# dsteinberg/libcluster

Hardware: AMD Instinct MI355X
Metric: E-step data-points/sec (full VBEM iteration: suff-stats + M-step + E-step) (higher is better)
Workload: dtype f64

## Files before the change

### libcluster_amd/csrc/lc_kernels.h

```cpp
#pragma once
#include <hip/hip_runtime.h>
#include <cstdint>

namespace lck {

constexpr int RG = 16;

inline int padded_dim(int D) {
  return D <= 16 ? 16 : D <= 32 ? 32 : D <= 48 ? 48 : D <= 64 ? 64 : D <= 80 ? 80 : D <= 96 ? 96 : D <= 112 ? 112 : D <= 128 ? 128 : -1;
}
__host__ __device__ constexpr int lds_row_stride(int DP) { return DP == 16 ? 16 : (DP + 16) % 32 != 16 ? DP + 32 : DP + 16; }
inline int padded_dim_wide(int D) { return D <= 128 ? padded_dim(D) : (D + 63) / 64 * 64; }
constexpr int GW_MAX_DP = 1024;
inline int ntiles(int DP) { int nt = DP / 4; return nt * (nt + 1) / 2; }
inline int pstride(int DP) { return ntiles(DP) * 16 + DP; }
constexpr int WIDE_CHUNK = 256 * 16 + 64;
inline int wide_chunks(int DP) { int np = DP / 64; return np * (np + 1) / 2; }
inline int64_t estep_pstride(int DP, int DC) { return DP > 128 ? (int64_t)wide_chunks(DP) * WIDE_CHUNK : (int64_t)pstride(DC); }
inline int64_t estep_pstride(int DP) { return estep_pstride(DP, DP); }
inline int estep_active_width(int D, int DP) {
  if (DP < 32 || DP > 128) return DP;
  const int g = DP <= 48 ? 4 : 8, lo = DP <= 48 ? DP - 12 : DP - 8;
  const int dc = (D + g - 1) / g * g;
  return dc < DP ? (dc < lo ? lo : dc) : DP;
}
inline int64_t stat_stride(int DP) { return 1 + (int64_t)DP + (int64_t)DP * DP; }

struct LdsGrant {
  size_t granted[16] = {};
};
inline hipError_t grant_dynamic_lds(const void* fn, size_t bytes, LdsGrant& g) {
  if (bytes <= 64 * 1024) return hipSuccess;
  int dev = -1;
  const bool tracked = hipGetDevice(&dev) == hipSuccess && dev >= 0 && dev < 16;
  if (tracked && bytes <= g.granted[dev]) return hipSuccess;
  const hipError_t e = hipFuncSetAttribute(fn, hipFuncAttributeMaxDynamicSharedMemorySize, (int)bytes);
  if (e == hipSuccess && tracked) g.granted[dev] = bytes;
  return e;
}

inline int rginfo_pack(int group, int nvalid) { return (group << 5) | nvalid; }

struct EstepLaunch {
  int DP;
  int DC = 0;
  const double* X;
  int64_t nrg;
  const int* rginfo;
  int64_t nrows;
  const double* params;
  const double* ctab;
  int K;
  double* qZ;
  int64_t ldq;
  double* fz_part;
  double* ll_part;
  int raw = 0;
  int sparse = 0;
  int lq_lds = 0;
};
struct EstepPlan {
  bool ok;
  int rows_per_block;
  int64_t grid;
  bool four_groups;
  int DC, lq_lds;
  size_t lds_bytes;
};
EstepPlan estep_plan(const EstepLaunch& a);
int64_t estep_grid(const EstepLaunch& a);
hipError_t launch_estep(const EstepLaunch& a, hipStream_t stream);

struct FusedLaunch {
  int DP;
  int D = 16;
  const double* X;
  int64_t nrg;
  const int* rginfo;
  int64_t nrows;
  const double* params;
  const double* ctab;
  int K;
  double* qZ;
  int64_t ldq;
  double* partial;
  bool want_ll;
  int grid;
  int ngroups = 1;
  int yshare = 0;
};
constexpr int FUSED_CT_CAP = 1024;
inline int64_t fused_record(int DP, int K) { return (int64_t)K * (1 + DP + (int64_t)DP * DP) + 1 + K; }
bool fused_eligible(int DP, int K);
int fused_plan(int DP, int64_t nrg, int K);
hipError_t launch_fused(const FusedLaunch& a, hipStream_t stream);

struct SSItem {
  int64_t r0, r1;
  int kofs, kcnt;
  int64_t rec0;
};
constexpr int SS_BR = 32;
constexpr double SPECK_TAU = 0x1p-300;
enum SuffstatRoute { SS_PER_CLUSTER = 0, SS_FEAT = 1, SS_QUAD = 2, SS_WIDE = 3 };
enum SuffstatMode { SS_DENSE = 0, SS_MASKED_DENSE = 1, SS_ZERO_SKIP = 2, SS_WORK_LIST = 3 };
struct SuffstatPlan {
  SuffstatRoute route;
  int nchunks;
  int64_t chunk_rows;
  int extra, klast0, KR;
  int clusters_per_block;
  const char* name;
};
SuffstatPlan suffstat_plan(int DP, int DC, int64_t NP, int K, SuffstatMode mode);
struct SuffstatLaunch {
  int DP;
  int DC = 0;
  const double* X;
  int64_t NP;
  const double* qZ;
  int64_t ldq;
  int K;
  SuffstatMode mode = SS_DENSE;
  const int* rginfo;
  const unsigned char* smask;
  double* partial;
  int nchunks = 0, KR = 0;
  int64_t chunk_rows = 0;
  const SSItem* items = nullptr;
  const int* klist = nullptr;
  int nitems = 0, skip_listed = 0;
  int speck_skip = 0;
  int nslice = 1;
  int slice0 = 0, rs = 1, klast0 = 0, nklast = 0;
  int64_t ldx = 0;
  int DPW = 0, colA = 0, colB = 0;
};
hipError_t launch_suffstat(const SuffstatLaunch& a, const SuffstatPlan& p, hipStream_t stream);

constexpr int SPECK_PROBE_STEPS = 4096;
constexpr int64_t SPECK_PROBE_MIN_ROWS = 4096;
hipError_t launch_speck_probe(const double* qZ, int64_t ldq, int K, int64_t NP, int* active, int64_t* pairs, hipStream_t stream,
                              int64_t* rows = nullptr);
inline bool speck_probe_says_skip(int64_t active, int64_t pairs) { return pairs > 0 && 4 * (pairs - active) >= pairs; }
bool speck_probe_says_lists(int64_t single, int64_t rows);

struct SsListLayout {
  int nq;
  bool wide;
  size_t ent_off;
  size_t bytes;
};
inline SsListLayout ss_list_layout(int nchunks, int64_t chunk_rows, int K) {
  SsListLayout l{(K + 3) / 4, chunk_rows > 65536, 0, 0};
  l.ent_off = ((size_t)nchunks * l.nq * sizeof(int) + 15) / 16 * 16;
  l.bytes = l.ent_off + (size_t)nchunks * l.nq * (size_t)chunk_rows * (l.wide ? 4 : 2);
  return l;
}
bool suffstat_list_instance(int DP, int DC);
bool speck_lists_enabled();
hipError_t launch_suffstat_list_build(const SuffstatLaunch& a, const SuffstatPlan& p, void* lists, size_t bytes, hipStream_t stream);
hipError_t launch_suffstat_lists(const SuffstatLaunch& a, const SuffstatPlan& p, void* lists, size_t bytes, hipStream_t stream);
int speck_skip_mode();

__host__ __device__ constexpr int ft_offdiag(int DC) { return (DC / 4) * (DC / 4 - 1) / 2; }
__host__ __device__ constexpr int ft_features(int DC) { return 16 * ft_offdiag(DC) + 10 * (DC / 4) + DC + 1; }
__host__ __device__ constexpr int ft_tiles(int DC) { return (ft_features(DC) + 15) / 16; }
enum FtKind { FT_PRODUCT = 0, FT_LINEAR = 1, FT_COUNT = 2, FT_SPARE = 3 };
struct FtFeature {
  int u, w, kind;
};
__host__ __device__ __attribute__((always_inline)) constexpr FtFeature ft_feature(int DC, int one, int f) {
  const int noff = 16 * ft_offdiag(DC), ndiag = 10 * (DC / 4);
  if (f < noff) {
    const int p = f / 16, r = f % 16;
    int ja = 1;
    while ((ja + 1) * ja / 2 <= p) ++ja;
    return {4 * (p - ja * (ja - 1) / 2) + (r & 3), 4 * ja + (r >> 2), FT_PRODUCT};
  }
  f -= noff;
  if (f < ndiag) {
    const int b = 4 * (f / 10), e = f % 10;
    const int i = e < 4 ? 0 : e < 7 ? 1 : e < 9 ? 2 : 3, i0 = e < 4 ? 0 : e < 7 ? 4 : e < 9 ? 7 : 9;
    return {b + i, b + i + (e - i0), FT_PRODUCT};
  }
  f -= ndiag;
  if (f < DC) return {f, one, FT_LINEAR};
  return {one, one, f == DC ? FT_COUNT : FT_SPARE};
}
#ifndef LC_FT_WAVES64
#define LC_FT_WAVES64 8
#endif
#ifndef LC_FT_WAVES128
#define LC_FT_WAVES128 8
#endif
__host__ __device__ constexpr int ft_waves(int DP) { return DP == 64 ? LC_FT_WAVES64 : DP == 128 ? LC_FT_WAVES128 : DP > 64 ? 8 : 4; }
__host__ __device__ constexpr int ft_tpw_max(int DP, int NQ) {
  const int t = (NQ >= 8 && DP > 64 && DP < 128 ? 64 : 72) / NQ;
  return t < 14 ? t : 14;
}
__host__ __device__ constexpr int ft_nslice(int DP, int DC, int NQ) {
  return (ft_tiles(DC) + ft_waves(DP) * ft_tpw_max(DP, NQ) - 1) / (ft_waves(DP) * ft_tpw_max(DP, NQ));
}
__host__ __device__ constexpr int ft_tpw(int DP, int DC, int NQ) {
  return (ft_tiles(DC) + ft_waves(DP) * ft_nslice(DP, DC, NQ) - 1) / (ft_waves(DP) * ft_nslice(DP, DC, NQ));
}
__host__ __device__ __attribute__((always_inline)) constexpr void ft_deal(int DP, int DC, int NQ, int slice, int wave, int* t0, int* nt) {
  const int tiles = ft_tiles(DC), nsl = ft_nslice(DP, DC, NQ);
  if (ft_waves(DP) == 8) {
    const int ns = 4 * nsl, s = slice * 4 + (wave & 3), l = tiles / ns, r = tiles % ns;
    const int load = l + (s < r ? 1 : 0), first = s * l + (s < r ? s : r);
    *t0 = first + (wave < 4 ? 0 : (load + 1) / 2);
    *nt = wave < 4 ? (load + 1) / 2 : load / 2;
  } else {
    const int tpw = ft_tpw(DP, DC, NQ), t = (slice * 4 + wave) * tpw;
    *t0 = t;
    *nt = tiles - t < tpw ? (tiles - t > 0 ? tiles - t : 0) : tpw;
  }
}
__host__ __device__ constexpr int ftl_tpw(int DC) { return ((ft_tiles(DC) + 3) / 4 + 1) / 2; }
__host__ __device__ __attribute__((always_inline)) constexpr void ft_deal_one(int DC, int wave, int* t0, int* nt) {
  const int tiles = ft_tiles(DC), s = wave & 3, l = tiles / 4, r = tiles % 4;
  const int load = l + (s < r ? 1 : 0), first = s * l + (s < r ? s : r);
  *t0 = first + (wave < 4 ? 0 : (load + 1) / 2);
  *nt = wave < 4 ? (load + 1) / 2 : load / 2;
}
__host__ __device__ constexpr int ft_nt_min(int DP, int DC, int NQ) {
  int m = ft_tpw(DP, DC, NQ);
  for (int sl = 0; sl < ft_nslice(DP, DC, NQ); ++sl)
    for (int w = 0; w < ft_waves(DP); ++w) {
      int t0 = 0, nt = 0;
      ft_deal(DP, DC, NQ, sl, w, &t0, &nt);
      m = nt < m ? nt : m;
    }
  return m;
}

hipError_t launch_fold_extra(double* rec, int64_t SS, int K, int klast0, int extra, hipStream_t stream);
hipError_t launch_reduce_records(const double* partial, int64_t n, int K, const int* kptr, const int* krec, double* out,
                                 hipStream_t stream);

constexpr int REDUCE_TMP_ELEMS = 512;
hipError_t launch_reduce_partials(const double* partial, int nparts, int64_t n, double* out, hipStream_t stream,
                                  double* tmp = nullptr);
hipError_t launch_group_colsum(const double* qZ, int64_t ldq, int K, const int64_t* goff, int J, double* out,
                               hipStream_t stream, double* tmp = nullptr, int64_t rows = 0);
hipError_t launch_fill_qz(double* qZ, int64_t ldq, int K, const int* rginfo, int64_t nrows, int64_t nrg, double value,
                          hipStream_t stream);
struct DiagEstepLaunch {
  int DP, D;
  const double* X;
  int64_t nrg;
  const int* rginfo;
  int64_t nrows;
  const double* params;
  int mode = 0;
  const double* ctab;
  int K;
  double* qZ;
  int64_t ldq;
  double* fz_part;
  double* ll_part;
  int raw = 0;
  const double* wt = nullptr;
  const double* mu = nullptr;
  const double* constk = nullptr;
  int ngroups = 1;
  double* sink = nullptr;
};
constexpr int EDM_CT_CAP = 1024;
inline int64_t estep_diag_grid(int64_t nrg) { return (nrg * RG + 63) / 64; }
int64_t estep_diag_mfma_weights(int DP, int K, int mode);
enum DiagEstepInstance { EDI_NONE = 0, EDI_GENERIC = 1, EDI_PLAIN = 2, EDI_TABLED = 3, EDI_ONEGROUP = 4 };
struct DiagEstepPlan {
  bool ok;
  bool mfma;
  int mode;
  int64_t grid;
  size_t lds_bytes;
  const char* name;
  bool wide;
  int KT;
  bool REG;
  int NT;
  bool QUAD;
  int R, KTM;
  int instance;
  int64_t nslots;
  int per_cu;
  int64_t block_cap;
};
DiagEstepPlan estep_diag_plan(const DiagEstepLaunch& a);
hipError_t launch_estep_diag(const DiagEstepLaunch& a, hipStream_t stream);
double estep_diag_centre(int D, int DP, int K, int mode, const double* a, const double* w2, double* mu);
void estep_diag_pack(int D, int DP, int K, int mode, const double* a, const double* w2, const double* w1, const double* mu,
                     double* constk, double* wt, int64_t nw);

struct DiagStatLaunch {
  int DP;
  const double* X;
  int64_t NP;
  const double* qZ;
  int64_t ldq;
  int K;
  const int* rginfo;
  const unsigned char* smask;
  double* partial;
  int nchunks;
  int64_t chunk_rows;
  int second = 1;
  int nslice = 0, rsplit = 0;
  int ldx = 0, col0 = 0, DPT = 0;
};
int suffstat_diag_rsplit(int K);
struct DiagStatPlan {
  bool ok;
  int nslice, rsplit;
  int second;
  int nblocks;
  int width, last_width;
  int BR, BR_last;
  bool nstage, nstage_last;
  bool deep, deep_last;
  size_t lds_bytes;
  const char* name;
};
DiagStatPlan suffstat_diag_plan(int DP, int K, int second);
hipError_t launch_suffstat_diag(const DiagStatLaunch& a, hipStream_t stream);

int select_blocks(int64_t NP);
hipError_t launch_select_count(const double* qcol, int64_t NP, double thresh, int* counts, hipStream_t stream);
hipError_t launch_select_compact(const double* qcol, int64_t NP, double thresh, const int64_t* offsets, int64_t* idx,
                                 hipStream_t stream);
hipError_t launch_group_starts(const int64_t* idx, int64_t M, const int64_t* goff, int J, int64_t* starts,
                               hipStream_t stream);
hipError_t launch_transpose_qz(const double* qZ, int64_t ldq, int K, int64_t NP, double* qT, hipStream_t stream);
hipError_t launch_gather_cols(const double* src, int64_t lds, int K, const int64_t* idx, int64_t M, const int64_t* starts,
                              const int64_t* goff_sub, int J, double* dst, int64_t ldd, hipStream_t stream);
hipError_t launch_gather_rowmajor(const double* src, int64_t lds, int K, const int64_t* idx, int64_t M,
                                  const int64_t* starts, const int64_t* goff_sub, int J, double* dst, int64_t ldd,
                                  hipStream_t stream);
hipError_t launch_gather_rowmajor_cols(const double* src, int64_t lds, const int* cols, int nc, const int64_t* idx, int64_t M,
                                       const int64_t* starts, const int64_t* goff_sub, int J, double* dst, int64_t ldd,
                                       hipStream_t stream);
hipError_t launch_gather_rows(const double* X, int DP, const int64_t* idx, int64_t M, const int64_t* starts,
                              const int64_t* goff_sub, int J, double* Xdst, hipStream_t stream);
hipError_t launch_split_init(const double* X, int DP, int D, int64_t NP, const int* rginfo, int64_t nrows,
                             const double* mv, double* q, int64_t ldq, int mode, const double* thr,
                             hipStream_t stream);
hipError_t launch_aug_from_sub(double* q, int64_t ldq, int k, int K, const int64_t* idx, int64_t M,
                               const int64_t* starts, const int64_t* goff_sub, int J, const double* qsub1,
                               hipStream_t stream, int64_t* qhash = nullptr);

struct CachedNormLaunch {
  const double* dcache;
  int64_t ldc;
  const double* fresh;
  int64_t ldf;
  const int* colmap;
  const double* ctab;
  int K;
  const int* rginfo;
  int64_t nrows, NP;
  double* qZ;
  int64_t ldq;
  double* fz_part;
  double* ll_part = nullptr;
  double* dq = nullptr;
  double dq_tol = 0.0;
  int64_t ldd = 0;
  double* amax = nullptr;
  int64_t* qhash = nullptr;
  int qhash_in = 0;
  double* rmax = nullptr;
  int* ramax = nullptr;
  unsigned long long* colmask = nullptr;
};
constexpr int BOUND_MAX_COLS = 8, BOUND_MAX_K = 72;
struct BoundSelectLaunch {
// ... 95 lines not shown
```

### libcluster_amd/csrc/lc_kernels_suffstat.hip

```cpp
#include "lc_device.hpp"

#ifndef LC_SS_FEAT_MINK_ACTIVE
#define LC_SS_FEAT_MINK_ACTIVE 5
#endif
#ifndef LC_SS_FEAT_WIDTHS
#define LC_SS_FEAT_WIDTHS(DP) ((DP) >= 32 && (DP) <= 128)
#endif

namespace lck {

template <int NB>
struct SSAcc { static constexpr int N = NB * 3 + NB * (NB - 1) / 2 * 4; };

template <int NB>
__host__ __device__ constexpr bool ss_in_half(int half, int jbp, int jb) {
  if (half == 0) return true;
  const bool first = NB == 8   ? (jbp < 5 || (jbp == 5 && jb < 3))
                     : NB == 7 ? (jbp < 4 || (jbp == 4 && jb < 4))
                     : NB == 6 ? (jbp < 4 || (jbp == 4 && jb < 1))
                               : (jbp == 1 || jbp == 2);
  return first == (half == 1);
}
template <int PAN>
constexpr int ss_batch_rows() { return PAN == 2 ? 24 : SS_BR; }
// ... 907 lines not shown
template <int DP, int DC, int NQ, bool SPECK>
static hipError_t launch_ss_feat_i(const SuffstatLaunch& b, hipStream_t stream) {
  constexpr int BR = ft_batch_rows(DP), LD = lds_row_stride(DP);
  const size_t shmem = (size_t)(2 * BR * LD + 2 * BR * ft_qld(NQ)) * sizeof(double);
  auto kern = suffstat_feat_kernel<DP, DC, NQ, SPECK>;
  static LdsGrant grant;
  if (hipError_t e = grant_dynamic_lds(reinterpret_cast<const void*>(kern), shmem, grant); e != hipSuccess) return e;
  hipLaunchKernelGGL(kern, dim3((unsigned)(b.nchunks * ft_nslice(DP, DC, NQ))), dim3(64 * ft_waves(DP)), shmem, stream, b);
  return hipGetLastError();
}
template <int DP, int DC, int NQ>
static hipError_t launch_ss_feat_q(const SuffstatLaunch& b, hipStream_t stream) {
  return b.speck_skip ? launch_ss_feat_i<DP, DC, NQ, true>(b, stream) : launch_ss_feat_i<DP, DC, NQ, false>(b, stream);
}
template <int DP, int DC>
static hipError_t launch_ss_feat_d(const SuffstatLaunch& a, hipStream_t stream) {
  SuffstatLaunch b = a;
  const int range = ft_range(DP, a.K);
  for (int k0 = 0; k0 < a.K; k0 += range) {
    b.klast0 = k0;
    const int nq = ((a.K - k0 < range ? a.K - k0 : range) + 3) / 4;
    hipError_t e = hipErrorInvalidValue;
    switch (ft_instance_quads(nq)) {
      case 2: e = launch_ss_feat_q<DP, DC, 2>(b, stream); break;
      case 4: e = launch_ss_feat_q<DP, DC, 4>(b, stream); break;
      case 5: e = launch_ss_feat_q<DP, DC, 5>(b, stream); break;
      case 6: e = launch_ss_feat_q<DP, DC, 6>(b, stream); break;
      case 7: e = launch_ss_feat_q<DP, DC, 7>(b, stream); break;
      case 8: e = launch_ss_feat_q<DP, DC, 8>(b, stream); break;
      case 16:
        if constexpr (DP == 128) e = launch_ss_feat_q<DP, DC, 16>(b, stream);
        break;
    }
    if (e != hipSuccess) return e;
  }
  return hipSuccess;
}
template <int DP>
static hipError_t launch_ss_feat_w(const SuffstatLaunch& a, hipStream_t stream) {
  if constexpr (DP <= 48) {
    if (a.DC == DP - 4) return launch_ss_feat_d<DP, DP - 4>(a, stream);
    if (a.DC == DP - 12) return launch_ss_feat_d<DP, DP - 12>(a, stream);
  }
  if (a.DC == DP - 8) return launch_ss_feat_d<DP, DP - 8>(a, stream);
  if (a.DC != 0 && a.DC != DP) return hipErrorInvalidValue;
  return launch_ss_feat_d<DP, DP>(a, stream);
}
static hipError_t launch_ss_feat(const SuffstatLaunch& a, hipStream_t stream) {
  switch (a.DP) {
    case 32: return launch_ss_feat_w<32>(a, stream);
    case 48: return launch_ss_feat_w<48>(a, stream);
    case 64: return launch_ss_feat_w<64>(a, stream);
    case 80: return launch_ss_feat_w<80>(a, stream);
    case 96: return launch_ss_feat_w<96>(a, stream);
    case 112: return launch_ss_feat_w<112>(a, stream);
    case 128: return launch_ss_feat_w<128>(a, stream);
  }
  return hipErrorInvalidValue;
}

#ifndef LC_FT_SPECK_LISTS
#define LC_FT_SPECK_LISTS 1
#endif
#ifndef LC_FTL_BR
#define LC_FTL_BR 48
#endif
bool speck_lists_enabled() { return LC_FT_SPECK_LISTS != 0; }
#ifndef LC_FT_LIST_SHARE64
#define LC_FT_LIST_SHARE64 58
#endif
bool speck_probe_says_lists(int64_t single, int64_t rows) { return rows > 0 && 64 * single >= (int64_t)LC_FT_LIST_SHARE64 * rows; }
bool suffstat_list_instance(int DP, int DC) { return DP == 64 && (DC == 0 || DC == 64 || DC == 56); }

template <typename IT>
__global__ void __launch_bounds__(256) ss_list_build_kernel(const double* __restrict__ qZ, int64_t ldq, int K, int64_t NP,
                                                             int64_t chunk_rows, int nq, int* __restrict__ lens, IT* __restrict__ ent) {
  __shared__ int wcnt[2][32][4];
  const int chunk = blockIdx.x, tid = threadIdx.x, lane = tid & 63, wave = tid >> 6;
  const int64_t r0 = (int64_t)chunk * chunk_rows;
  const int64_t r1 = (r0 + chunk_rows) < NP ? (r0 + chunk_rows) : NP;
  if (r0 >= r1) {
    for (int c = tid; c < nq; c += 256) lens[(int64_t)chunk * nq + c] = 0;
    return;
  }
  for (int q0 = 0; q0 < nq; q0 += 32) {
    const int nqg = nq - q0 < 32 ? nq - q0 : 32;
    int base = 0, par = 0;
    for (int64_t t0 = r0; t0 < r1; t0 += 256, par ^= 1) {
      const int64_t row = t0 + tid;
      const bool valid = row < r1;
      const double* qr = qZ + (valid ? row : r1 - 1);
      unsigned m = 0;
      for (int c8 = 0; c8 < nqg; c8 += 8) {
        double v[32];
#pragma unroll
        for (int i = 0; i < 32; ++i) {
          const int k = 4 * (q0 + c8) + i;
          v[i] = qr[(int64_t)(k < K ? k : K - 1) * ldq];
        }
#pragma unroll
        for (int i = 0; i < 32; ++i) {
          const int k = 4 * (q0 + c8) + i;
          if (valid && k < K && !(v[i] < SPECK_TAU)) m |= 1u << (c8 + i / 4);
        }
      }
      int mycnt = 0;
      for (int c = 0; c < nqg; ++c) {
        const unsigned long long bal = __ballot((m >> c) & 1u);
        if (lane == c) mycnt = __popcll(bal);
      }
      if (lane < nqg) wcnt[par][lane][wave] = mycnt;
      __syncthreads();
      int mybase = 0;
      if (lane < nqg) {
        int tot = 0, before = 0;
#pragma unroll
        for (int w = 0; w < 4; ++w) {
          const int n = wcnt[par][lane][w];
          before += w < wave ? n : 0;
          tot += n;
        }
        mybase = base + before;
        base += tot;
      }
      for (int c = 0; c < nqg; ++c) {
        const unsigned long long bal = __ballot((m >> c) & 1u);
        const int at = __shfl(mybase, c) + (int)__builtin_amdgcn_mbcnt_hi((unsigned)(bal >> 32), __builtin_amdgcn_mbcnt_lo((unsigned)bal, 0u));
        if ((m >> c) & 1u) ent[((int64_t)chunk * nq + q0 + c) * chunk_rows + at] = (IT)(row - r0);
      }
    }
    if (wave == 0 && lane < nqg) lens[(int64_t)chunk * nq + q0 + lane] = base;
    __syncthreads();
  }
}

template <int DP, int DC, typename IT>
__global__ void __launch_bounds__(512, 2) suffstat_list_kernel(SuffstatLaunch a, const int* __restrict__ lens, const IT* __restrict__ ent,
                                                                int nq) {
  static_assert(DC % 4 == 0 && DC <= DP && DC > DP - 16, "active width");
  constexpr int NTHR = 512, BR = LC_FTL_BR, LD = lds_row_stride(DP), QLD = 4, XBUF = BR * LD, QBUF = BR * QLD;
  constexpr int ONE = DP, NT = ftl_tpw(DC);
  constexpr int TPR = DP / 2, RPP = NTHR / TPR, NPRE = BR / RPP;
  static_assert(LD > DP && NTHR % TPR == 0 && BR % RPP == 0 && BR % 4 == 0 && 4 * BR <= NTHR, "staging");
  static_assert((XBUF + (BR - 4) * LD + LD) * 8 <= 65536, "fragment reads: one address register per tile, the rest immediate");
  extern __shared__ __attribute__((aligned(16))) double lds[];
  double* xbuf = lds;
  double* qbuf = lds + 2 * XBUF;
  const int tid = threadIdx.x, lane = tid & 63, wave = tid >> 6;
  const int hi = lane >> 4, blk = (lane >> 2) & 3, lo2 = lane & 3;
  const int chunk = blockIdx.x / nq, quad = blockIdx.x % nq;
  const int64_t r0 = (int64_t)chunk * a.chunk_rows;
  const int len = lens[blockIdx.x];
  const IT* li = ent + (int64_t)blockIdx.x * a.chunk_rows;
  int T0 = 0, nt = 0;
  ft_deal_one(DC, wave, &T0, &nt);
  const double* pu[NT];
  const double* pw[NT];
#pragma unroll
  for (int t = 0; t < NT; ++t) {
    const FtFeature f = t < nt ? ft_feature(DC, ONE, 16 * (T0 + t) + lo2 + 4 * blk) : FtFeature{ONE, ONE, FT_SPARE};
    pu[t] = xbuf + hi * LD + f.u;
    pw[t] = xbuf + hi * LD + f.w;
  }
  double acc[NT];
#pragma unroll
  for (int t = 0; t < NT; ++t) acc[t] = 0.0;

  const int xr0 = tid / TPR, xc2 = tid % TPR, qrow = tid / 4, qcl = tid % 4;
  const bool qthr = tid < 4 * BR;
  const int kq = 4 * quad + qcl;
  const double* qcol = a.qZ + (int64_t)(kq < a.K ? kq : a.K - 1) * a.ldq + r0;
  int xi[NPRE], qi = -1;
  double pre[NPRE][2], qpre = 0.0;
  auto iload = [&](int p0) {
#pragma unroll
    for (int i = 0; i < NPRE; ++i) {
      const int p = p0 + xr0 + i * RPP;
      xi[i] = p < len ? (int)li[p] : -1;
    }
    qi = qthr && p0 + qrow < len ? (int)li[p0 + qrow] : -1;
  };
  auto gload = [&]() {
#pragma unroll
    for (int i = 0; i < NPRE; ++i) {
      const double2 v = *reinterpret_cast<const double2*>(a.X + (r0 + (xi[i] < 0 ? 0 : xi[i])) * DP + 2 * xc2);
      pre[i][0] = xi[i] < 0 ? 0.0 : v.x;
      pre[i][1] = xi[i] < 0 ? 0.0 : v.y;
    }
    const double q = qcol[qi < 0 ? 0 : qi];
    qpre = qi < 0 || kq >= a.K ? 0.0 : q;
  };
  auto lstore = [&](int buf) {
#pragma unroll
    for (int i = 0; i < NPRE; ++i)
      *reinterpret_cast<double2*>(xbuf + buf * XBUF + (xr0 + i * RPP) * LD + 2 * xc2) = make_double2(pre[i][0], pre[i][1]);
    if (qthr) qbuf[buf * QBUF + qrow * QLD + qcl] = qpre;
  };
  if (tid < 2 * BR) xbuf[(tid / BR) * XBUF + (tid % BR) * LD + ONE] = 1.0;
  if (len > 0) {
    iload(0);
    gload();
    iload(BR);
    lstore(0);
  }
  __syncthreads();
  const double* pq = qbuf + hi * QLD + lo2;
  auto batch = [&](auto bsel) {
    constexpr int B = decltype(bsel)::value, XO = B * XBUF, QO = B * QBUF;
    double uf[NT], wf[NT], pp[NT];
#pragma unroll
    for (int t = 0; t < NT; ++t) {
      uf[t] = pu[t][XO];
      wf[t] = pw[t][XO];
    }
    double qa = pq[QO];
#pragma unroll
    for (int st = 0; st < BR / 4; ++st) {
#pragma unroll
      for (int t = 0; t < NT; ++t) pp[t] = uf[t] * wf[t];
      const double qc = qa;
      if (st + 1 < BR / 4) {
#pragma unroll
        for (int t = 0; t < NT; ++t) {
          uf[t] = pu[t][XO + (st + 1) * 4 * LD];
          wf[t] = pw[t][XO + (st + 1) * 4 * LD];
        }
        qa = pq[QO + (st + 1) * 4 * QLD];
      }
      __builtin_amdgcn_sched_barrier(0);
#pragma unroll
      for (int t = 0; t < NT; ++t) acc[t] = mfma4(qc, pp[t], acc[t]);
      __builtin_amdgcn_sched_barrier(0);
    }
  };
  for (int p0 = 0; p0 < len; p0 += 2 * BR) {
    const bool more1 = p0 + BR < len, more2 = p0 + 2 * BR < len;
    if (more1) {
      gload();
      iload(p0 + 2 * BR);
    }
    batch(std::integral_constant<int, 0>{});
    if (more1) lstore(1);
    __syncthreads();
    if (!more1) break;
    if (more2) {
      gload();
      iload(p0 + 3 * BR);
    }
    batch(std::integral_constant<int, 1>{});
    if (more2) lstore(0);
    __syncthreads();
  }

  const int64_t SS = 1 + (int64_t)DP + (int64_t)DP * DP;
  int wv = wave, T0e = 0, nte = 0;
  asm volatile("" : "+v"(wv));
  ft_deal_one(DC, wv, &T0e, &nte);
  const int kk = 4 * quad + hi;
  if (kk >= a.K) return;
  double* out = a.partial + ((int64_t)chunk * a.KR + kk) * SS;
#pragma unroll
  for (int t = 0; t < NT; ++t) {
    if (t >= nte) continue;
    const FtFeature f = ft_feature(DC, ONE, 16 * (T0e + t) + lo2 + 4 * blk);
    if (f.kind == FT_SPARE) continue;
    const double v = acc[t];
    if (f.kind == FT_PRODUCT) {
      double* S = out + 1 + DP;
      S[(int64_t)f.u * DP + f.w] = v;
      S[(int64_t)f.w * DP + f.u] = v;
    } else if (f.kind == FT_LINEAR) {
      out[1 + f.u] = v;
    } else {
      out[0] = v;
    }
  }
}

static hipError_t ss_list_check(const SuffstatLaunch& a, const SuffstatPlan& p, const void* lists, size_t bytes, SsListLayout* lay) {
  if (a.K <= 0 || p.nchunks <= 0 || !lists || !a.qZ || !a.X) return hipErrorInvalidValue;
  if (p.route != SS_FEAT || a.mode != SS_DENSE || a.smask || a.items || p.extra != 0) return hipErrorInvalidValue;
  if (a.nchunks != p.nchunks || a.chunk_rows != p.chunk_rows || a.KR != p.KR || a.KR != a.K) return hipErrorInvalidValue;
  if (!suffstat_list_instance(a.DP, a.DC)) return hipErrorInvalidValue;
  if (a.chunk_rows < 4 || a.chunk_rows % 4 || a.chunk_rows > (int64_t)1 << 30 || (int64_t)a.nchunks * a.chunk_rows < a.NP) return hipErrorInvalidValue;
  *lay = ss_list_layout(a.nchunks, a.chunk_rows, a.K);
  if ((int64_t)a.nchunks * lay->nq > (int64_t)1 << 30 || bytes < lay->bytes) return hipErrorInvalidValue;
  return hipSuccess;
}
hipError_t launch_suffstat_list_build(const SuffstatLaunch& a, const SuffstatPlan& p, void* lists, size_t bytes, hipStream_t stream) {
  SsListLayout lay;
  if (hipError_t e = ss_list_check(a, p, lists, bytes, &lay); e != hipSuccess) return e;
  int* lens = static_cast<int*>(lists);
  void* ent = static_cast<char*>(lists) + lay.ent_off;
  if (lay.wide)
    hipLaunchKernelGGL(ss_list_build_kernel<unsigned>, dim3((unsigned)a.nchunks), dim3(256), 0, stream, a.qZ, a.ldq, a.K, a.NP,
                       a.chunk_rows, lay.nq, lens, static_cast<unsigned*>(ent));
  else
    hipLaunchKernelGGL(ss_list_build_kernel<unsigned short>, dim3((unsigned)a.nchunks), dim3(256), 0, stream, a.qZ, a.ldq, a.K, a.NP,
                       a.chunk_rows, lay.nq, lens, static_cast<unsigned short*>(ent));
  return hipGetLastError();
}
template <int DP, int DC, typename IT>
static hipError_t launch_ss_list_i(const SuffstatLaunch& a, const SsListLayout& lay, const void* lists, hipStream_t stream) {
  constexpr int BR = LC_FTL_BR;
  const size_t shmem = (size_t)(2 * BR * lds_row_stride(DP) + 2 * BR * 4) * sizeof(double);
  auto kern = suffstat_list_kernel<DP, DC, IT>;
  static LdsGrant grant;
  if (hipError_t e = grant_dynamic_lds(reinterpret_cast<const void*>(kern), shmem, grant); e != hipSuccess) return e;
  hipLaunchKernelGGL(kern, dim3((unsigned)(a.nchunks * lay.nq)), dim3(512), shmem, stream, a, static_cast<const int*>(lists),
                     reinterpret_cast<const IT*>(static_cast<const char*>(lists) + lay.ent_off), lay.nq);
  return hipGetLastError();
}
hipError_t launch_suffstat_lists(const SuffstatLaunch& a, const SuffstatPlan& p, void* lists, size_t bytes, hipStream_t stream) {
  SsListLayout lay;
  if (hipError_t e = ss_list_check(a, p, lists, bytes, &lay); e != hipSuccess) return e;
  if (hipError_t e = launch_suffstat_list_build(a, p, lists, bytes, stream); e != hipSuccess) return e;
  const bool narrow = a.DC == 56;
  if (lay.wide) return narrow ? launch_ss_list_i<64, 56, unsigned>(a, lay, lists, stream) : launch_ss_list_i<64, 64, unsigned>(a, lay, lists, stream);
  return narrow ? launch_ss_list_i<64, 56, unsigned short>(a, lay, lists, stream)
                : launch_ss_list_i<64, 64, unsigned short>(a, lay, lists, stream);
}

struct SqItem {
  int kind, ia, ja;
};
__host__ __device__ constexpr int sq_items(int DC) { return (DC / 4) * (DC / 4 + 1) / 2 + DC / 4 + 1; }
__host__ __device__ constexpr SqItem sq_item(int DC, int n) {
  for (int ja = 0; ja < DC / 4; ++ja) {
    if (n <= ja) return SqItem{0, n, ja};
    n -= ja + 1;
    if (n == 0) return SqItem{1, 0, ja};
    n -= 1;
  }
  return SqItem{2, 0, 0};
}
__host__ __device__ constexpr int sq_part_lo(int DC, int NPART, int p) { return (sq_items(DC) * p + NPART - 1) / NPART; }
__host__ __device__ constexpr int sq_part_max(int DC, int NPART) {
  int m = 0;
  for (int p = 0; p < NPART; ++p) {
    const int n = sq_part_lo(DC, NPART, p + 1) - sq_part_lo(DC, NPART, p);
    m = n > m ? n : m;
  }
  return m;
}
constexpr int SQ_BR = 32, SQ_QLD = 18;
inline int sq_npart(int DP, int K) {
  const int nq = (K + 3) / 4;
  if (DP > 48) return 4;
  return nq == 2 ? 2 : nq == 4 ? (DP <= 32 ? 1 : 2) : 4;
}
inline int sq_nslice(int DP, int K) { return (((K + 3) / 4) * sq_npart(DP, K) + 3) / 4; }
inline bool ss_quad_eligible(int DP, int K) {
  static const int mode = test_switch("LC_SS_QUAD") ? atoi(test_switch("LC_SS_QUAD")) : -1;
  if (mode == 0 || DP < 32 || DP > 64 || K < 1 || K > 16) return false;
  if (mode == 1) return true;
  return K >= 3;
}
template <int DP, int DC, int NPART>
__global__ void __launch_bounds__(256, 2) suffstat_quad_kernel(SuffstatLaunch a) {
  static_assert(DC % 4 == 0 && DC <= DP && DC > DP - 16, "active width");
  constexpr int NT = DC / 4, BR = SQ_BR, LD = lds_row_stride(DP), QLD = SQ_QLD, XBUF = BR * LD, QBUF = BR * QLD, NTHR = 256;
  constexpr int NACC = sq_part_max(DC, NPART);
  extern __shared__ __attribute__((aligned(16))) double lds[];
  double* xbuf = lds;
  double* qbuf = lds + 2 * XBUF;
  const int tid = threadIdx.x, lane = tid & 63, wave = tid >> 6;
  const int hi = lane >> 4, blk = (lane >> 2) & 3, lo2 = lane & 3;
  const int K = a.K, NQ = (K + 3) / 4;
  int chunk, slice;
  {
    const int nslice = a.nslice, nchunks = a.nchunks, b = blockIdx.x, full = (nchunks / 8) * 8;
    if (b < full * nslice) {
      const int xcd = b & 7, seq = b >> 3;
      chunk = (seq / nslice) * 8 + xcd;
      slice = seq % nslice;
    } else {
      const int t = b - full * nslice;
      chunk = full + t / nslice;
      slice = t % nslice;
    }
  }
  const int64_t r0 = (int64_t)chunk * a.chunk_rows;
  const int64_t r1 = (r0 + a.chunk_rows) < a.NP ? (r0 + a.chunk_rows) : a.NP;
  const int unit = slice * 4 + wave, quad = unit / NPART, part = unit % NPART;
  const bool busy = quad < NQ;

  constexpr int TPR = DP / 2, NV2 = BR * TPR, NPRE = (NV2 + NTHR - 1) / NTHR;
  double pre[NPRE][2], qpre[4];
  const int qcl = tid % 16, qrq = tid / 16;
  const bool qthr = qrq < BR / 4;
  auto gload = [&](int64_t b0) {
#pragma unroll
    for (int i = 0; i < NPRE; ++i) {
      const int idx = tid + i * NTHR;
      const int row = idx / TPR, c2 = idx % TPR;
      double2 v = make_double2(0.0, 0.0);
      if (row < BR && b0 + row < r1) v = *reinterpret_cast<const double2*>(a.X + (b0 + row) * DP + 2 * c2);
      pre[i][0] = v.x;
      pre[i][1] = v.y;
    }
    const int64_t qrow = b0 + 4 * qrq;
#pragma unroll
    for (int i = 0; i < 4; ++i) qpre[i] = 0.0;
    if (qthr && qcl < K && qrow < r1) {
      const double2* qp = reinterpret_cast<const double2*>(a.qZ + (int64_t)qcl * a.ldq + qrow);
      const double2 v0 = qp[0], v1 = qp[1];
      qpre[0] = v0.x, qpre[1] = v0.y, qpre[2] = v1.x, qpre[3] = v1.y;
    }
  };
  auto lstore = [&](int buf) {
#pragma unroll
    for (int i = 0; i < NPRE; ++i) {
      const int idx = tid + i * NTHR;
      const int row = idx / TPR, c2 = idx % TPR;
      if (row < BR) *reinterpret_cast<double2*>(xbuf + buf * XBUF + row * LD + 2 * c2) = make_double2(pre[i][0], pre[i][1]);
    }
    if (qthr) {
// ... 386 lines not shown
```

### libcluster_amd/csrc/lc_testhooks.hip

```cpp
#include <algorithm>
#include <cstdio>
#include <vector>

#include "lc_device.hpp"
#include "lc_predict.hpp"

namespace {

using lck::RG;
typedef long long i64;

class Scope {
 public:
  ~Scope() {
    for (auto& b : bufs_)
      if (b.d) (void)hipFree(b.d);
  }
  template <typename T>
  T* in(const T* h, size_t n) { return static_cast<T*>(add(const_cast<T*>(h), n * sizeof(T), false, true)); }
  template <typename T>
  T* io(T* h, size_t n) { return static_cast<T*>(add(h, n * sizeof(T), true, true)); }
  template <typename T>
  T* out(T* h, size_t n) { return static_cast<T*>(add(h, n * sizeof(T), true, false)); }
  template <typename T>
// ... 641 lines not shown
  if (m == lck::SS_MASKED_DENSE && !smask) return -1;
  if (masked && (!rginfo || J < 1 || J > (1 << 20) || !rginfo_ok(rginfo, NP / RG, J))) return -1;
  if (fold && (!folded || nfolded < (i64)K * lck::stat_stride(DP))) return -1;
  const lck::SuffstatPlan p = lck::suffstat_plan(DP, DC, NP, K, m);
  plan_out[0] = p.route, plan_out[1] = p.nchunks, plan_out[2] = p.chunk_rows, plan_out[3] = p.extra, plan_out[4] = p.klast0;
  plan_out[5] = p.KR, plan_out[6] = p.clusters_per_block;
  if (p.nchunks < 1 || p.chunk_rows < lck::SS_BR || p.chunk_rows % lck::SS_BR || (i64)p.nchunks * p.chunk_rows < NP) return -1;
  const i64 SS = lck::stat_stride(DP);
  i64 nrec = (i64)p.nchunks * p.KR;
  std::vector<lck::SSItem> items;
  std::vector<int> kptr, krec;
  if (listed) {
    if (!r0 || !r1 || !kofs || !kcnt || !rec0 || !klist || nitems < 1 || nklist < 1 || nrec_listed < 1) return -1;
    nrec = nrec_listed;
    for (int t = 0; t < nklist; ++t)
      if (klist[t] < 0 || klist[t] >= K) return -1;
    std::vector<char> used((size_t)nrec, 0);
    std::vector<std::vector<int>> recs((size_t)K);
    for (int i = 0; i < nitems; ++i) {
      if (r0[i] < 0 || r0[i] > r1[i] || r1[i] > NP || r0[i] % RG || r1[i] % RG) return -1;
      if (kcnt[i] < 1 || kcnt[i] > p.clusters_per_block || kofs[i] < 0 || kofs[i] > nklist - kcnt[i]) return -1;
      if (rec0[i] < 0 || rec0[i] > nrec - kcnt[i]) return -1;
      for (int t = 0; t < kcnt[i]; ++t) {
        if (used[(size_t)(rec0[i] + t)]) return -1;
        used[(size_t)(rec0[i] + t)] = 1;
        recs[(size_t)klist[kofs[i] + t]].push_back((int)(rec0[i] + t));
      }
      items.push_back(lck::SSItem{r0[i], r1[i], kofs[i], kcnt[i], rec0[i]});
    }
    kptr.assign((size_t)K + 1, 0);
    for (int k = 0; k < K; ++k) {
      krec.insert(krec.end(), recs[(size_t)k].begin(), recs[(size_t)k].end());
      kptr[(size_t)k + 1] = (int)krec.size();
    }
  }
  if (npartial < nrec * SS) return -1;
  Scope s;
  lck::SuffstatLaunch a{};
  a.DP = DP;
  a.DC = DC;
  a.X = s.in(X, (size_t)NP * DP);
  a.NP = NP;
  a.qZ = s.in(qZ, (size_t)K * (size_t)ldq);
  a.ldq = ldq;
  a.K = K;
  a.mode = m;
  a.rginfo = masked ? s.in(rginfo, (size_t)(NP / RG)) : nullptr;
  a.smask = masked ? s.in(smask, (size_t)J * K) : nullptr;
  a.partial = s.io(partial, (size_t)npartial);
  a.nchunks = p.nchunks;
  a.KR = p.KR;
  a.chunk_rows = p.chunk_rows;
  a.speck_skip = speck_skip < 0 ? (p.route == lck::SS_FEAT ? lck::speck_skip_mode() : 0) : speck_skip;
  const int* dkptr = nullptr;
  const int* dkrec = nullptr;
  if (listed) {
    a.items = s.in(items.data(), items.size());
    a.klist = s.in(klist, (size_t)nklist);
    a.nitems = nitems;
    a.skip_listed = skip_listed ? 1 : 0;
    if (fold) {
      dkptr = s.in(kptr.data(), kptr.size());
      dkrec = s.in(krec.data(), krec.size());
    }
  }
  double* dfold = fold ? s.io(folded, (size_t)nfolded) : nullptr;
  double* ext = fold && !listed && p.extra > 0 ? s.scratch<double>((size_t)p.KR * (size_t)SS) : nullptr;
  if (!s.ok()) return s.finish(hipSuccess);
  hipError_t e = lck::launch_suffstat(a, p, nullptr);
  if (e == hipSuccess && fold) {
    if (listed) {
      e = lck::launch_reduce_records(a.partial, SS, K, dkptr, dkrec, dfold, nullptr);
    } else if (p.extra > 0) {
      e = lck::launch_reduce_partials(a.partial, p.nchunks, (i64)p.KR * SS, ext, nullptr);
      if (e == hipSuccess) e = lck::launch_fold_extra(ext, SS, K, p.klast0, p.extra, nullptr);
      if (e == hipSuccess) e = hipMemcpyAsync(dfold, ext, (size_t)K * (size_t)SS * sizeof(double), hipMemcpyDeviceToDevice, nullptr);
    } else {
      e = lck::launch_reduce_partials(a.partial, p.nchunks, (i64)K * SS, dfold, nullptr);
    }
  }
  return s.finish(e);
}
LC_HOOK lc_test_suffstat(const double* X, int DP, int DC, i64 NP, const double* qZ, int K, i64 ldq, int mode, const int* rginfo,
                         const unsigned char* smask, int J, int nitems, const i64* r0, const i64* r1, const int* kofs, const int* kcnt,
                         const i64* rec0, const int* klist, int nklist, int nrec_listed, int skip_listed, double* partial, i64 npartial,
                         int fold, double* folded, i64 nfolded, i64* plan_out) {
  return test_suffstat(X, DP, DC, NP, qZ, K, ldq, mode, rginfo, smask, J, nitems, r0, r1, kofs, kcnt, rec0, klist, nklist, nrec_listed,
                       skip_listed, partial, npartial, fold, folded, nfolded, plan_out, -1);
}
LC_HOOK lcx_test_suffstat_speck(const double* X, int DP, int DC, i64 NP, const double* qZ, int K, i64 ldq, int mode, const int* rginfo,
                                const unsigned char* smask, int J, int nitems, const i64* r0, const i64* r1, const int* kofs,
                                const int* kcnt, const i64* rec0, const int* klist, int nklist, int nrec_listed, int skip_listed,
                               double* partial, i64 npartial, int fold, double* folded, i64 nfolded, i64* plan_out, int speck_skip) {
  if (speck_skip < 0 || speck_skip > 2) return -1;
  return test_suffstat(X, DP, DC, NP, qZ, K, ldq, mode, rginfo, smask, J, nitems, r0, r1, kofs, kcnt, rec0, klist, nklist, nrec_listed,
                       skip_listed, partial, npartial, fold, folded, nfolded, plan_out, speck_skip);
}

LC_HOOK lcx_test_suffstat_lists(const double* X, int DP, int DC, i64 NP, const double* qZ, int K, i64 ldq, int sums, double* partial,
                                i64 npartial, int fold, double* folded, i64 nfolded, i64* plan_out, int* lens_out, i64 nlens, int* ent_out,
                                i64 nent) {
  if (!X || !qZ || !partial || !plan_out || !lens_out || !ent_out || K < 1 || K > 4096 || !gw_width_ok(DP, DC)) return -1;
  if (NP < RG || NP % RG || NP > HOT_MAX_NRG * RG || ldq < NP || ldq % 2) return -1;
  const i64 SS = lck::stat_stride(DP);
  if (fold && (!sums || !folded || nfolded < (i64)K * SS)) return -1;
  const lck::SuffstatPlan p = lck::suffstat_plan(DP, DC, NP, K, lck::SS_DENSE);
  plan_out[0] = p.route, plan_out[1] = p.nchunks, plan_out[2] = p.chunk_rows, plan_out[3] = p.extra, plan_out[4] = p.klast0;
  plan_out[5] = p.KR, plan_out[6] = p.clusters_per_block;
  if (p.nchunks < 1 || p.chunk_rows < lck::SS_BR || p.chunk_rows % lck::SS_BR || (i64)p.nchunks * p.chunk_rows < NP) return -1;
  const lck::SsListLayout lay = lck::ss_list_layout(p.nchunks, p.chunk_rows, K);
  const i64 nseg = (i64)p.nchunks * lay.nq;
  if (npartial < (i64)p.nchunks * p.KR * SS || nlens < nseg || nent < nseg * p.chunk_rows) return -1;
  Scope s;
  lck::SuffstatLaunch a{};
  a.DP = DP;
  a.DC = DC;
  a.X = s.in(X, (size_t)NP * DP);
  a.NP = NP;
  a.qZ = s.in(qZ, (size_t)K * (size_t)ldq);
  a.ldq = ldq;
  a.K = K;
  a.mode = lck::SS_DENSE;
  a.rginfo = nullptr;
  a.smask = nullptr;
  a.partial = s.io(partial, (size_t)npartial);
  a.nchunks = p.nchunks;
  a.KR = p.KR;
  a.chunk_rows = p.chunk_rows;
  unsigned char* lists = s.scratch<unsigned char>(lay.bytes);
  double* dfold = fold ? s.io(folded, (size_t)nfolded) : nullptr;
  if (!s.ok()) return s.finish(hipSuccess);
  hipError_t e = hipMemset(lists, 0xff, lay.bytes);
  if (e == hipSuccess)
    e = sums ? lck::launch_suffstat_lists(a, p, lists, lay.bytes, nullptr) : lck::launch_suffstat_list_build(a, p, lists, lay.bytes, nullptr);
  if (e == hipSuccess && fold) e = lck::launch_reduce_partials(a.partial, p.nchunks, (i64)K * SS, dfold, nullptr);
  const int rc = s.finish(e);
  if (rc != 0) return rc;
  std::vector<unsigned char> raw(lay.bytes);
  if (hipMemcpy(raw.data(), lists, lay.bytes, hipMemcpyDeviceToHost) != hipSuccess) return -1;
  const int* lens = reinterpret_cast<const int*>(raw.data());
  for (i64 g = 0; g < nseg; ++g)
    if (lens[g] < 0 || lens[g] > p.chunk_rows) return -2;
  for (i64 g = 0; g < nseg; ++g) {
    lens_out[g] = lens[g];
    for (int i = 0; i < lens[g]; ++i) {
      const size_t at = (size_t)g * (size_t)p.chunk_rows + (size_t)i;
      ent_out[at] = lay.wide ? (int)reinterpret_cast<const unsigned*>(raw.data() + lay.ent_off)[at]
                             : (int)reinterpret_cast<const unsigned short*>(raw.data() + lay.ent_off)[at];
    }
  }
  return 0;
}

LC_HOOK lc_test_fused_plan(int DP, i64 nrg, int K, i64* out) {
  if (!out || K < 1 || K > 4096 || nrg < 0 || nrg > HOT_MAX_NRG || DP < 1 || DP > 1024) return -1;
  out[0] = lck::fused_eligible(DP, K) ? 1 : 0;
  out[1] = lck::fused_plan(DP, nrg, K);
  out[2] = lck::current_device_cus();
  out[3] = (i64)lck::fused_record(DP, K);
  return 0;
}
LC_HOOK lc_test_fused(const double* X, int D, i64 nrg, const double* params, const double* ctab, int J, const int* rginfo, i64 nrows,
                      int K, int want_ll, int grid, double* qZ, int Kbuf, i64 ldq, double* partial, i64 npartial, int* grid_used) {
  const int DP = 16;
  if (!X || !params || !ctab || !qZ || !partial || !grid_used || D < 1 || D > DP || K < 1 || Kbuf < K || Kbuf > 8192) return -1;
  if (nrg < 1 || nrg > HOT_MAX_NRG || ldq < nrg * RG || J < 1 || J > (1 << 20) || !lck::fused_eligible(DP, K)) return -1;
  if (rginfo ? !rginfo_ok(rginfo, nrg, J) : (J != 1 || nrows < 0 || nrows > nrg * RG)) return -1;
  const int plan = lck::fused_plan(DP, nrg, K);
  if (plan < 1 || grid < 0 || grid > plan) return -1;
  const int g = grid ? grid : plan;
  if (npartial < (i64)g * lck::fused_record(DP, K)) return -1;
  *grid_used = g;
  Scope s;
  lck::FusedLaunch a{};
  a.DP = DP;
  a.D = D;
  a.X = s.in(X, (size_t)(nrg * RG) * DP);
  a.nrg = nrg;
  a.rginfo = rginfo ? s.in(rginfo, (size_t)nrg) : nullptr;
  a.nrows = nrows;
  a.params = s.in(params, (size_t)K * (size_t)lck::pstride(DP));
  a.ctab = s.in(ctab, (size_t)J * K);
  a.K = K;
  a.qZ = s.io(qZ, (size_t)Kbuf * (size_t)ldq);
  a.ldq = ldq;
  a.partial = s.io(partial, (size_t)npartial);
  a.want_ll = want_ll != 0;
  a.grid = g;
  a.ngroups = J;
  if (!s.ok()) return s.finish(hipSuccess);
  return s.finish(lck::launch_fused(a, nullptr));
}

namespace {

bool diag_width_ok(int DP) { return DP >= 16 && (DP <= 128 ? DP % 16 == 0 : (DP % 64 == 0 && DP <= 1024)); }

void diag_estep_plan_out(const lck::DiagEstepPlan& p, i64* out, char* name) {
  out[0] = p.ok ? 1 : 0, out[1] = p.mfma ? 1 : 0, out[2] = p.mode, out[3] = p.grid, out[4] = (i64)p.lds_bytes;
  out[5] = p.wide ? 1 : 0, out[6] = p.KT, out[7] = p.REG ? 1 : 0, out[8] = p.NT, out[9] = p.QUAD ? 1 : 0, out[10] = p.R;
  out[11] = p.KTM, out[12] = p.instance, out[13] = p.nslots, out[14] = p.per_cu, out[15] = p.block_cap;
  if (name) snprintf(name, 32, "%s", p.name ? p.name : "");
}
void diag_stat_plan_out(const lck::DiagStatPlan& p, i64* out, char* name) {
  out[0] = p.ok ? 1 : 0, out[1] = p.nslice, out[2] = p.rsplit, out[3] = p.second, out[4] = p.nblocks, out[5] = p.width;
  out[6] = p.last_width, out[7] = p.BR, out[8] = p.BR_last, out[9] = p.nstage ? 1 : 0, out[10] = p.nstage_last ? 1 : 0;
  out[11] = p.deep ? 1 : 0, out[12] = p.deep_last ? 1 : 0, out[13] = (i64)p.lds_bytes;
  if (name) snprintf(name, 32, "%s", p.name ? p.name : "");
}
constexpr int DIAG_SINK = 256, DIAG_SINK_GUARD = 64;

}

LC_HOOK lc_test_estep_diag_plan(int DP, int K, int mode, i64 nrg, int mfma, int raw, int want_ll, int grouped, int ngroups,
                                i64* out, char* name) {
  if (!out || !name || K < 1 || K > 4096 || nrg < 0 || nrg > HOT_MAX_NRG || DP < 1 || DP > 1024 || mode < 0 || mode > 2 || ngroups < 1)
    return -1;
  static double some;
  static int somei;
  lck::DiagEstepLaunch a{};
  a.DP = DP, a.D = DP, a.K = K, a.mode = mode, a.nrg = nrg, a.raw = raw ? 1 : 0, a.ngroups = ngroups;
  a.wt = mfma ? &some : nullptr;
  a.ll_part = want_ll ? &some : nullptr;
  a.rginfo = grouped ? &somei : nullptr;
  diag_estep_plan_out(lck::estep_diag_plan(a), out, name);
  return 0;
}
LC_HOOK lc_test_estep_diag(const double* X, int DP, i64 nrg, const double* params, int mode, const double* ctab, int J,
                           const int* rginfo, i64 nrows, int K, int raw, const double* wt, i64 nwt, const double* mu,
                           const double* constk, double* qZ, int Kbuf, i64 ldq, double* fz_part, i64 nfz, double* ll_part, i64 nll,
                           double* sink, i64* plan_out, char* name) {
  if (!X || !params || !ctab || !qZ || !fz_part || !plan_out || !name || K < 1 || K > 4096 || Kbuf < K || Kbuf > 8192) return -1;
  if (J < 1 || J > (1 << 20) || mode < 0 || mode > 2 || nrg < 1 || nrg > HOT_MAX_NRG || nrg * RG > ldq) return -1;
  if (!diag_width_ok(DP)) return -1;
  if (rginfo ? !rginfo_ok(rginfo, nrg, J) : (J != 1 || nrows < 0 || nrows > nrg * RG)) return -1;
  if (wt) {
    const i64 nw = lck::estep_diag_mfma_weights(DP, K, mode);
    if (nw <= 0 || nwt != nw || !constk || !sink || (mode != 2 && !mu)) return -1;
  } else if (nwt != 0 || mu || constk || sink) {
    return -1;
  }
  lck::DiagEstepLaunch a{};
  a.DP = DP, a.D = DP, a.K = K, a.mode = mode, a.nrg = nrg, a.nrows = nrows, a.raw = raw ? 1 : 0, a.ngroups = J, a.ldq = ldq;
  static double some;
  a.wt = wt ? &some : nullptr;
  a.ll_part = ll_part ? &some : nullptr;
  a.rginfo = rginfo;
  const lck::DiagEstepPlan p = lck::estep_diag_plan(a);
  diag_estep_plan_out(p, plan_out, name);
  if (!p.ok || p.grid < 1 || p.grid > p.nslots || p.lds_bytes > HOT_LDS_LIMIT) return -1;
  if (nfz < p.nslots || (ll_part && nll < p.nslots * K)) return -1;
  Scope s;
  a.X = s.in(X, (size_t)(nrg * RG) * DP);
  a.params = s.in(params, (size_t)3 * K * DP);
  a.ctab = s.in(ctab, (size_t)J * K);
  a.rginfo = rginfo ? s.in(rginfo, (size_t)nrg) : nullptr;
  a.qZ = s.io(qZ, (size_t)Kbuf * (size_t)ldq);
  a.fz_part = s.io(fz_part, (size_t)nfz);
  a.ll_part = ll_part ? s.io(ll_part, (size_t)nll) : nullptr;
  a.wt = nullptr;
  if (wt) {
    a.wt = s.in(wt, (size_t)nwt);
    std::vector<double> zero((size_t)DP, 0.0);
    a.mu = s.in(mu ? mu : zero.data(), (size_t)DP);
    a.constk = s.in(constk, (size_t)K);
    a.sink = s.io(sink, (size_t)(DIAG_SINK + DIAG_SINK_GUARD));
  }
  if (!s.ok()) return s.finish(hipSuccess);
  return s.finish(lck::launch_estep_diag(a, nullptr));
}

LC_HOOK lc_test_suffstat_diag_plan(int DP, int K, int second, i64* out, char* name) {
  if (!out || !name) return -1;
  diag_stat_plan_out(lck::suffstat_diag_plan(DP, K, second), out, name);
  return 0;
}
LC_HOOK lc_test_suffstat_diag(const double* X, int DP, i64 NP, const double* qZ, int K, i64 ldq, const int* rginfo,
                              const unsigned char* smask, int J, int nchunks, i64 chunk_rows, int second, double* partial,
                              i64 npartial, int fold, double* folded, i64 nfolded, i64* plan_out) {
  if (!X || !qZ || !partial || !plan_out || K < 1 || K > 4096 || !diag_width_ok(DP)) return -1;
  if (NP < RG || NP % RG || NP > HOT_MAX_NRG * RG || ldq < NP) return -1;
  if (nchunks < 1 || chunk_rows < 32 || chunk_rows % 32 || chunk_rows > HOT_MAX_NRG * RG) return -1;
  if (!((i64)(nchunks - 1) * chunk_rows < NP && NP <= (i64)nchunks * chunk_rows)) return -1;
  if ((smask != nullptr) != (rginfo != nullptr)) return -1;
  if (smask && (J < 1 || J > (1 << 20) || !rginfo_ok(rginfo, NP / RG, J))) return -1;
  const lck::DiagStatPlan p = lck::suffstat_diag_plan(DP, K, second);
  diag_stat_plan_out(p, plan_out, nullptr);
  if (!p.ok || p.lds_bytes > HOT_LDS_LIMIT) return -1;
  const i64 SS = 1 + 2 * (i64)DP;
  const i64 nparts = (i64)nchunks * p.rsplit;
  if (npartial < nparts * K * SS || nparts > (1 << 24)) return -1;
  if (fold && (!folded || nfolded < (i64)K * SS)) return -1;
  Scope s;
  lck::DiagStatLaunch a{};
  a.DP = DP;
  a.X = s.in(X, (size_t)NP * DP);
  a.NP = NP;
  a.qZ = s.in(qZ, (size_t)K * (size_t)ldq);
  a.ldq = ldq;
  a.K = K;
  a.rginfo = smask ? s.in(rginfo, (size_t)(NP / RG)) : nullptr;
  a.smask = smask ? s.in(smask, (size_t)J * K) : nullptr;
  a.partial = s.io(partial, (size_t)npartial);
  a.nchunks = nchunks;
  a.chunk_rows = chunk_rows;
  a.second = second ? 1 : 0;
// ... 20 lines not shown
```

Measured before the change: 358.4 million.

## Share w-operand fragments across off-diagonal tiles in list suffstat kernel for DC=64

For active width 64, the list-based sufficient-statistics kernel now deals feature tiles so each wave owns two column blocks ("stars"). The off-diagonal product tiles in a star then share the same w-column, so each wave loads only a few distinct w fragments from LDS per row batch instead of one per tile. This is meant to cut LDS read traffic and register pressure in the inner outer-product loop. It adds a new feature-to-wave mapping, scheduling barriers, and a test hook, with the risk that the changed deal unbalances work or breaks the correctness of the output write-back.

```diff
diff --git a/libcluster_amd/csrc/lc_kernels.h b/libcluster_amd/csrc/lc_kernels.h
--- a/libcluster_amd/csrc/lc_kernels.h
+++ b/libcluster_amd/csrc/lc_kernels.h
@@ -170,23 +170,26 @@
 struct FtFeature {
   int u, w, kind;
 };
+__host__ __device__ __attribute__((always_inline)) constexpr FtFeature ft_feature_rest(int DC, int one, int g) {
+  const int ndiag = 10 * (DC / 4);
+  if (g < ndiag) {
+    const int b = 4 * (g / 10), e = g % 10;
+    const int i = e < 4 ? 0 : e < 7 ? 1 : e < 9 ? 2 : 3, i0 = e < 4 ? 0 : e < 7 ? 4 : e < 9 ? 7 : 9;
+    return {b + i, b + i + (e - i0), FT_PRODUCT};
+  }
+  g -= ndiag;
+  if (g < DC) return {g, one, FT_LINEAR};
+  return {one, one, g == DC ? FT_COUNT : FT_SPARE};
+}
 __host__ __device__ __attribute__((always_inline)) constexpr FtFeature ft_feature(int DC, int one, int f) {
-  const int noff = 16 * ft_offdiag(DC), ndiag = 10 * (DC / 4);
+  const int noff = 16 * ft_offdiag(DC);
   if (f < noff) {
     const int p = f / 16, r = f % 16;
     int ja = 1;
     while ((ja + 1) * ja / 2 <= p) ++ja;
     return {4 * (p - ja * (ja - 1) / 2) + (r & 3), 4 * ja + (r >> 2), FT_PRODUCT};
   }
-  f -= noff;
-  if (f < ndiag) {
-    const int b = 4 * (f / 10), e = f % 10;
-    const int i = e < 4 ? 0 : e < 7 ? 1 : e < 9 ? 2 : 3, i0 = e < 4 ? 0 : e < 7 ? 4 : e < 9 ? 7 : 9;
-    return {b + i, b + i + (e - i0), FT_PRODUCT};
-  }
-  f -= ndiag;
-  if (f < DC) return {f, one, FT_LINEAR};
-  return {one, one, f == DC ? FT_COUNT : FT_SPARE};
+  return ft_feature_rest(DC, one, f - noff);
 }
 #ifndef LC_FT_WAVES64
 #define LC_FT_WAVES64 8
@@ -225,6 +228,39 @@
   *t0 = first + (wave < 4 ? 0 : (load + 1) / 2);
   *nt = wave < 4 ? (load + 1) / 2 : load / 2;
 }
+#ifndef LC_FTL_SHARED
+#define LC_FTL_SHARED 1
+#endif
+__host__ __device__ constexpr bool ftl_shared(int DC) { return LC_FTL_SHARED != 0 && DC == 64; }
+__host__ __device__ constexpr int ftl_paired(int DC) { return ftl_shared(DC) ? DC / 4 - 1 : 0; }
+__host__ __device__ constexpr int ftl_split(int DC) { return ftl_shared(DC) ? DC / 8 : 0; }
+struct FtlFeature {
+  int u, w, kind;
+  int shared;
+};
+__host__ __device__ __attribute__((always_inline)) constexpr FtlFeature ftl_feature(int DC, int one, int wave, int t, int l16) {
+  if (!ftl_shared(DC)) {
+    int t0 = 0, nt = 0;
+    ft_deal_one(DC, wave, &t0, &nt);
+    if (t >= nt) return {one, one, FT_SPARE, -1};
+    const FtFeature f = ft_feature(DC, one, 16 * (t0 + t) + l16);
+    return {f.u, f.w, f.kind, -1};
+  }
+  const int nb = DC / 4, S = ftl_split(DC), P = ftl_paired(DC);
+  if (t < P) {
+    const int second = t >= S ? 1 : 0, a = wave + second * S, o = (a + 1 + t - second * S) % nb;
+    return {4 * o + (l16 & 3), 4 * a + (l16 >> 2), FT_PRODUCT, second};
+  }
+  const FtFeature f = ft_feature_rest(DC, one, 16 * (2 * wave + t - P) + l16);
+  return {f.u, f.w, f.kind, -1};
+}
+__host__ __device__ constexpr int ftl_nw(int DC) { return ftl_shared(DC) ? 2 + ftl_tpw(DC) - ftl_paired(DC) : ftl_tpw(DC); }
+__host__ __device__ constexpr int ftl_wi(int DC, int t) {
+  return !ftl_shared(DC) ? t : t < ftl_split(DC) ? 0 : t < ftl_paired(DC) ? 1 : 2 + t - ftl_paired(DC);
+}
+static_assert(!ftl_shared(64) || (ftl_tpw(64) == ftl_paired(64) + 2 && 16 * 2 * 8 >= ft_features(64) - 16 * ft_offdiag(64)),
+              "shared deal: 8 waves of two stars and two free tiles");
+
 __host__ __device__ constexpr int ft_nt_min(int DP, int DC, int NQ) {
   int m = ft_tpw(DP, DC, NQ);
   for (int sl = 0; sl < ft_nslice(DP, DC, NQ); ++sl)
diff --git a/libcluster_amd/csrc/lc_kernels_suffstat.hip b/libcluster_amd/csrc/lc_kernels_suffstat.hip
--- a/libcluster_amd/csrc/lc_kernels_suffstat.hip
+++ b/libcluster_amd/csrc/lc_kernels_suffstat.hip
@@ -1083,15 +1083,16 @@
   const int64_t r0 = (int64_t)chunk * a.chunk_rows;
   const int len = lens[blockIdx.x];
   const IT* li = ent + (int64_t)blockIdx.x * a.chunk_rows;
-  int T0 = 0, nt = 0;
-  ft_deal_one(DC, wave, &T0, &nt);
+  constexpr int NW = ftl_nw(DC);
   const double* pu[NT];
-  const double* pw[NT];
+  const double* pw[NW];
 #pragma unroll
   for (int t = 0; t < NT; ++t) {
-    const FtFeature f = t < nt ? ft_feature(DC, ONE, 16 * (T0 + t) + lo2 + 4 * blk) : FtFeature{ONE, ONE, FT_SPARE};
+    const FtlFeature f = ftl_feature(DC, ONE, wave, t, lo2 + 4 * blk);
     pu[t] = xbuf + hi * LD + f.u;
-    pw[t] = xbuf + hi * LD + f.w;
+    int ow = hi * LD + f.w;
+    if constexpr (ftl_shared(DC)) asm volatile("" : "+v"(ow));
+    pw[ftl_wi(DC, t)] = xbuf + ow;
   }
   double acc[NT];
 #pragma unroll
@@ -1138,24 +1139,23 @@
   const double* pq = qbuf + hi * QLD + lo2;
   auto batch = [&](auto bsel) {
     constexpr int B = decltype(bsel)::value, XO = B * XBUF, QO = B * QBUF;
-    double uf[NT], wf[NT], pp[NT];
-#pragma unroll
-    for (int t = 0; t < NT; ++t) {
-      uf[t] = pu[t][XO];
-      wf[t] = pw[t][XO];
-    }
+    double uf[NT], wf[NW], pp[NT];
+#pragma unroll
+    for (int t = 0; t < NT; ++t) uf[t] = pu[t][XO];
+#pragma unroll
+    for (int i = 0; i < NW; ++i) wf[i] = pw[i][XO];
     double qa = pq[QO];
+    if constexpr (ftl_shared(DC)) __builtin_amdgcn_sched_barrier(0);
 #pragma unroll
     for (int st = 0; st < BR / 4; ++st) {
 #pragma unroll
-      for (int t = 0; t < NT; ++t) pp[t] = uf[t] * wf[t];
+      for (int t = 0; t < NT; ++t) pp[t] = uf[t] * wf[ftl_wi(DC, t)];
       const double qc = qa;
       if (st + 1 < BR / 4) {
 #pragma unroll
-        for (int t = 0; t < NT; ++t) {
-          uf[t] = pu[t][XO + (st + 1) * 4 * LD];
-          wf[t] = pw[t][XO + (st + 1) * 4 * LD];
-        }
+        for (int t = 0; t < NT; ++t) uf[t] = pu[t][XO + (st + 1) * 4 * LD];
+#pragma unroll
+        for (int i = 0; i < NW; ++i) wf[i] = pw[i][XO + (st + 1) * 4 * LD];
         qa = pq[QO + (st + 1) * 4 * QLD];
       }
       __builtin_amdgcn_sched_barrier(0);
@@ -1184,16 +1184,14 @@
   }
 
   const int64_t SS = 1 + (int64_t)DP + (int64_t)DP * DP;
-  int wv = wave, T0e = 0, nte = 0;
+  int wv = wave;
   asm volatile("" : "+v"(wv));
-  ft_deal_one(DC, wv, &T0e, &nte);
   const int kk = 4 * quad + hi;
   if (kk >= a.K) return;
   double* out = a.partial + ((int64_t)chunk * a.KR + kk) * SS;
 #pragma unroll
   for (int t = 0; t < NT; ++t) {
-    if (t >= nte) continue;
-    const FtFeature f = ft_feature(DC, ONE, 16 * (T0e + t) + lo2 + 4 * blk);
+    const FtlFeature f = ftl_feature(DC, ONE, wv, t, lo2 + 4 * blk);
     if (f.kind == FT_SPARE) continue;
     const double v = acc[t];
     if (f.kind == FT_PRODUCT) {
diff --git a/libcluster_amd/csrc/lc_testhooks.hip b/libcluster_amd/csrc/lc_testhooks.hip
--- a/libcluster_amd/csrc/lc_testhooks.hip
+++ b/libcluster_amd/csrc/lc_testhooks.hip
@@ -817,6 +817,22 @@
   return 0;
 }
 
+LC_HOOK lcx_test_suffstat_list_deal(int DP, int DC, i64* info, int* feat, i64 nfeat) {
+  if (!info || !feat || !gw_width_ok(DP, DC) || !lck::suffstat_list_instance(DP, DC)) return -1;
+  const int dc = DC ? DC : DP, waves = 8, tiles = lck::ftl_tpw(dc);
+  if (nfeat < (i64)waves * tiles * 16 * 4) return -1;
+  info[0] = lck::ftl_shared(dc) ? 1 : 0, info[1] = waves, info[2] = tiles, info[3] = lck::ftl_paired(dc), info[4] = lck::ftl_split(dc);
+  info[5] = DP;
+  for (int v = 0; v < waves; ++v)
+    for (int t = 0; t < tiles; ++t)
+      for (int l = 0; l < 16; ++l) {
+        const lck::FtlFeature f = lck::ftl_feature(dc, DP, v, t, l);
+        int* o = feat + ((size_t)(v * tiles + t) * 16 + l) * 4;
+        o[0] = f.u, o[1] = f.w, o[2] = f.kind, o[3] = f.shared;
+      }
+  return 0;
+}
+
 LC_HOOK lc_test_fused_plan(int DP, i64 nrg, int K, i64* out) {
   if (!out || K < 1 || K > 4096 || nrg < 0 || nrg > HOT_MAX_NRG || DP < 1 || DP > 1024) return -1;
   out[0] = lck::fused_eligible(DP, K) ? 1 : 0;
```

New measurement: 376.3 million, median of 6. +5.0%, better.
